# gregspangenberg/shoulder

Hardware: AMD Instinct MI355X
Metric: humerus meshes/s end-to-end (all 4 landmarks) (higher is better)
Workload: dtype f64 geometry + bf16 UNet

## Files before the change

### shoulder_amd/csrc/k_unet16_pp.h

```cpp
#pragma once
#include <type_traits>
#include "k_unet16_base.h"

namespace sh {

#define PP_THREADS 512
#define PP_GTHREADS 256
#define PP_NPIECE 11
#define PP_BUFB (PP_NPIECE * 4096)
#define PP_K1 11
#define PP_G1PRIO 0
#define PP_OFFPRIO 0

template <int N> __device__ inline void pp_wait_vm() {
  if constexpr (N == 0) asm volatile("s_waitcnt vmcnt(0)" ::: "memory");
  else if constexpr (N == 1) asm volatile("s_waitcnt vmcnt(1)" ::: "memory");
  else if constexpr (N == 2) asm volatile("s_waitcnt vmcnt(2)" ::: "memory");
  else if constexpr (N == 3) asm volatile("s_waitcnt vmcnt(3)" ::: "memory");
  else if constexpr (N == 4) asm volatile("s_waitcnt vmcnt(4)" ::: "memory");
  else if constexpr (N == 5) asm volatile("s_waitcnt vmcnt(5)" ::: "memory");
  else if constexpr (N == 6) asm volatile("s_waitcnt vmcnt(6)" ::: "memory");
  else if constexpr (N == 7) asm volatile("s_waitcnt vmcnt(7)" ::: "memory");
  else if constexpr (N == 8) asm volatile("s_waitcnt vmcnt(8)" ::: "memory");
  else if constexpr (N == 9) asm volatile("s_waitcnt vmcnt(9)" ::: "memory");
// ... 634 lines not shown
  const int xh = wv & 1, rg4 = wv >> 1;
  const int ltid = tid & (PP_GTHREADS - 1);
  const int H2 = H >> 1, W2 = W >> 1;
  const int tiles_x = W / 32, tiles_y = H / 8;
  if (tid == 0) { s_q[0] = ud_take_ticket(ticket); s_q[1] = ud_take_ticket(ticket); }

  for (int e = tid; e < 2 * 9 * 32 * 4; e += PP_THREADS) {
    const int row = e >> 2, q = e & 3;
    const int cc = row / 288, rem = row - cc * 288, tap = rem >> 5, j = rem & 31;
    const int ch = 8 * ((j & 15) >> 2) + 4 * (j >> 4) + (j & 3);
    *(u32x4*)(smem + DA_W + e * 16) = *(const u32x4*)(wgt + (size_t)((tap * 2 + cc) * 32 + ch) * 32 + ((q ^ ((row >> 1) & 2)) << 3));
  }
  v8 uw[2][2];
  f32x4 bv[2], ub[2];
#pragma unroll
  for (int kc = 0; kc < 2; ++kc)
#pragma unroll
    for (int n = 0; n < 2; ++n) {
      u32x4 t = *(const u32x4*)(wup + (size_t)((wv * 2 + kc) * 32 + 8 * (li >> 2) + 4 * n + (li & 3)) * 32 + 8 * lk);
      pp_settle(t);
      uw[kc][n] = __builtin_bit_cast(v8, t);
    }
#pragma unroll
  for (int n = 0; n < 2; ++n) {
#pragma unroll
    for (int r = 0; r < 4; ++r) { bv[n][r] = bias[8 * lk + 4 * n + r]; ub[n][r] = upb[8 * lk + 4 * n + r]; }
    pp_settle(bv[n]); pp_settle(ub[n]);
  }
  __syncthreads();
  const int t0 = __builtin_amdgcn_readfirstlane(s_q[0]);
  asm volatile("s_waitcnt vmcnt(0) lgkmcnt(0)" ::: "memory");
  __syncthreads();

  PpCursor cu;
  if (t0 >= ntk) return;
  auto decode = [&](int w) __attribute__((always_inline)) { cu.ty = w % tiles_y; w /= tiles_y; cu.tx = w % tiles_x; cu.img = w / tiles_x; };
  cu.w = tk_tab[t0]; cu.wend = tk_tab[t0 + 1]; cu.qk = 1; cu.live = true;
  decode(cu.w);
  auto advance = [&](const bool fetcher) __attribute__((always_inline)) {
    if (cu.w + 1 < cu.wend) { ++cu.w; if (++cu.ty == tiles_y) { cu.ty = 0; if (++cu.tx == tiles_x) { cu.tx = 0; ++cu.img; } } return; }
    const int nt = __builtin_amdgcn_readfirstlane(s_q[cu.qk]);
    if (nt < ntk) {
      if (fetcher) s_q[cu.qk ^ 1] = ud_take_ticket(ticket);
      cu.qk ^= 1;
      cu.w = tk_tab[nt]; cu.wend = tk_tab[nt + 1];
      decode(cu.w);
    } else cu.live = false;
  };

  const unsigned lds0 = __builtin_amdgcn_readfirstlane((unsigned)(size_t)(ud_lptr)smem);
  const unsigned wv1024 = (unsigned)(wv * 1024);
  int svoff[DA_NSP], lvoff[DA_NLP];
  const int sq8 = ((ltid & 3) ^ (((ltid >> 2) >> 1) & 2)) * 8;
#pragma unroll
  for (int k = 0; k < DA_NSP; ++k) {
    const int r = (ltid >> 2) + 64 * k, py = r / UD_PW, px = r - py * UD_PW;
    svoff[k] = (r < DA_ROWS && px < 34) ? ((py * W + px) * 32 + sq8) * 2 : ((W + 1) * 32 + sq8) * 2;
  }
#pragma unroll
  for (int k = 0; k < DA_NLP; ++k) {
    const int e = ltid + 256 * k, c = e >= 4 * DA_LROWS ? 1 : 0, rem = e - c * 4 * DA_LROWS, lr = rem >> 2;
    const int a = lr / 18, b = lr - a * 18;
    lvoff[k] = (c * (H2 * W2) + a * W2 + b) * 64 + (((rem & 3) ^ ((lr >> 1) & 2)) << 4);
  }
  const bool s5 = (ltid >> 2) + 64 * 5 < DA_ROWS, l3 = ltid + 256 * 3 < 2 * 4 * DA_LROWS;
  auto stage_skip = [&](int bf) __attribute__((always_inline)) {
    const ET* simg = skip + (size_t)cu.img * H * W * 32;
    const unsigned lb = lds0 + (unsigned)(bf * DA_HB) + wv1024;
    if (cu.tx > 0 && cu.tx + 1 < tiles_x && cu.ty > 0 && cu.ty + 1 < tiles_y) {
      const ET* base = simg + ((size_t)(cu.ty * 8 - 1) * W + (cu.tx * 32 - 1)) * 32;
#pragma unroll
      for (int k = 0; k < DA_NSP; ++k)
        if (k < DA_NSP - 1 || s5) ud_dma16_s(lb + k * 4096, (unsigned)svoff[k], base);
    } else {
#pragma unroll
      for (int k = 0; k < DA_NSP; ++k) {
        const int r = (ltid >> 2) + 64 * k, py = r / UD_PW, px = r - py * UD_PW;
        const int gx = cu.tx * 32 + px - 1, gy = cu.ty * 8 + py - 1;
        const bool ok = px < 34 && gx >= 0 && gx < W && gy >= 0 && gy < H;
        const ET* p = ok ? simg + (unsigned)((gy * W + gx) * 32 + sq8) : zero_page;
        if (k < DA_NSP - 1 || s5) ud_dma16(lb + k * 4096, p);
      }
    }
  };
  auto stage_low = [&](int bf) __attribute__((always_inline)) {
    const ET* limg = low + (size_t)cu.img * H2 * W2 * 64;
    const unsigned lb = lds0 + (unsigned)(DA_LOW + bf * DA_LB) + wv1024;
    if (cu.tx > 0 && cu.tx + 1 < tiles_x && cu.ty > 0 && cu.ty + 1 < tiles_y) {
      const ET* base = limg + ((size_t)(cu.ty * 4 - 1) * W2 + (cu.tx * 16 - 1)) * 32;
#pragma unroll
      for (int k = 0; k < DA_NLP; ++k)
        if (k < DA_NLP - 1 || l3) ud_dma16_s(lb + k * 4096, (unsigned)lvoff[k], base);
    } else {
#pragma unroll
      for (int k = 0; k < DA_NLP; ++k) {
        const int e = ltid + 256 * k, c = e >= 4 * DA_LROWS ? 1 : 0, rem = e - c * 4 * DA_LROWS, lr = rem >> 2;
        const int a = lr / 18, b = lr - a * 18;
        const int ly = cu.ty * 4 - 1 + a, lx = cu.tx * 16 - 1 + b;
        const bool ok = ly >= 0 && ly < H2 && lx >= 0 && lx < W2;
        const ET* p = ok ? limg + (size_t)c * H2 * W2 * 32 + (unsigned)((ly * W2 + lx) * 32 + (((rem & 3) ^ ((lr >> 1) & 2)) << 3)) : zero_page;
        if (k < DA_NLP - 1 || l3) ud_dma16(lb + k * 4096, p);
      }
    }
  };
  const int pdy = wv >> 1, pdx = wv & 1;
  int u_low[6], u_out[6];
#pragma unroll
  for (int g = 0; g < 6; ++g) {
    const int t = 16 * g + li;
    const bool valid = t < 85;
    const int a = valid ? t / 17 : 0, bc = valid ? t - a * 17 : 0;
    const int lowrow = (a + (pdy == 0 ? 1 : 0)) * 18 + bc + (pdx == 0 ? 1 : 0);
    const int py = 2 * a + (pdy == 0 ? 1 : 0), px = 2 * bc + (pdx == 0 ? 1 : 0);
    u_low[g] = UB_OFF(lowrow, lk) * 2;
    u_out[g] = valid ? UB_OFF(py * UD_PW + px, lk) * 2 : -1;
  }
  auto upconv = [&](int lb, int ub_, int x0, int y0) __attribute__((always_inline)) {
    const bool interior = x0 > 0 && x0 + 32 < W && y0 > 0 && y0 + 8 < H;
    const unsigned char* lp = smem + DA_LOW + lb * DA_LB;
    unsigned char* op = smem + DA_UP + ub_ * DA_HB;
#pragma unroll
    for (int g0 = 0; g0 < 6; g0 += 3) {
      v8 xf[3][2];
#pragma unroll
      for (int g = 0; g < 3; ++g)
#pragma unroll
        for (int kc = 0; kc < 2; ++kc) xf[g][kc] = *(const v8*)(lp + kc * (DA_LROWS * 64) + u_low[g0 + g]);
      f32x4 ua[3][2];
#pragma unroll
      for (int g = 0; g < 3; ++g)
#pragma unroll
        for (int n = 0; n < 2; ++n) {
          ua[g][n] = ub[n];
#pragma unroll
          for (int kc = 0; kc < 2; ++kc) ua[g][n] = E16<ET>::mfma(uw[kc][n], xf[g][kc], ua[g][n]);
        }
#pragma unroll
      for (int g = 0; g < 3; ++g) {
        u32x4 o;
#pragma unroll
        for (int n = 0; n < 2; ++n) {
          const f32x2 a01 = {ua[g][n][0], ua[g][n][1]}, a23 = {ua[g][n][2], ua[g][n][3]};
          o[2 * n] = __builtin_bit_cast(unsigned, __builtin_convertvector(a01, v2));
          o[2 * n + 1] = __builtin_bit_cast(unsigned, __builtin_convertvector(a23, v2));
        }
        if (!interior) {
          const int t = 16 * (g0 + g) + li, a = t / 17, bc = t - a * 17;
          const int gy = y0 - 1 + 2 * a + (pdy == 0 ? 1 : 0), gx = x0 - 1 + 2 * bc + (pdx == 0 ? 1 : 0);
          if (!(gy >= 0 && gy < H && gx >= 0 && gx < W)) o = u32x4{0u, 0u, 0u, 0u};
        }
        if (u_out[g0 + g] >= 0) *(u32x4*)(op + u_out[g0 + g]) = o;
      }
    }
  };
  int xoff[2][3];
  {
    const int rowbase = rg4 * 4 * UD_PW + xh * 16 + li;
#pragma unroll
    for (int sp = 0; sp < 2; ++sp)
#pragma unroll
      for (int dx = 0; dx < 3; ++dx) xoff[sp][dx] = UB_OFF(rowbase + sp * UD_PW + dx, lk) * 2;
  }
  const int woff = UB_OFF(li, lk) * 2;
  const unsigned so_lane = (unsigned)(((rg4 * 4) * W + xh * 16 + li) * 32 + 8 * lk);

  int ax0 = 0, ay0 = 0, aimg = 0;
  int bx0, by0, bimg; bool blive;
  int cx0, cy0, cimg; bool clive;
  bool alive = false;
  bx0 = cu.tx * 32; by0 = cu.ty * 8; bimg = cu.img; blive = true;
  if (grp == 0) stage_low(0); else stage_skip(0);
  advance(tid == 0);
  asm volatile("s_waitcnt vmcnt(0) lgkmcnt(0)" ::: "memory");
  __builtin_amdgcn_s_barrier();
  asm volatile("" ::: "memory");
  cx0 = cu.tx * 32; cy0 = cu.ty * 8; cimg = cu.img; clive = cu.live;
  if (grp == 0 && cu.live) stage_low(1);
  if (grp == 1) upconv(0, 0, bx0, by0);
  if (cu.live) advance(tid == 0);
  asm volatile("s_waitcnt vmcnt(0) lgkmcnt(0)" ::: "memory");
  __builtin_amdgcn_s_barrier();
  asm volatile("" ::: "memory");

  f32x4 acc[4][2];
#ifdef PP_STAMP
  unsigned long long st_[PP_NSTAMP] = {0, 0, 0, 0, 0, 0, 0, 0};
  PP_T(tl0_);
#endif
  int bf = 0;
  auto phase = [&](const bool on) __attribute__((always_inline)) -> bool {
    if (!blive && !alive) return false;
    PP_T(ta_);
    if (on) {
      if (blive) {
#pragma unroll
        for (int n = 0; n < 2; ++n)
#pragma unroll
          for (int m = 0; m < 4; ++m) acc[m][n] = bv[n];
        if (DA_ONPRIO) __builtin_amdgcn_s_setprio(DA_ONPRIO);
        const unsigned char* sb0 = smem + bf * DA_HB;
        const unsigned char* sb1 = smem + DA_UP + bf * DA_HB;
        const unsigned char* wbp = smem + DA_W + woff;
        v8 xq[2][6], wf[3][2];
        auto tap_of = [](int t) { const int g = t / 3, dy = t % 3; return (g / 3) * 9 + dy * 3 + g % 3; };
#pragma unroll
        for (int s = 0; s < 6; ++s) xq[0][s] = *(const v8*)(sb0 + xoff[s & 1][0] + (s & ~1) * UD_PW * 64);
#pragma unroll
        for (int t = 0; t < 2; ++t)
#pragma unroll
          for (int n = 0; n < 2; ++n) wf[t][n] = *(const v8*)(wbp + (tap_of(t) * 32 + n * 16) * 64);
#pragma unroll
        for (int t = 0; t < 18; ++t) {
          const int g = t / 3, dy = t % 3;
          if (dy == 0 && g + 1 < 6) {
            const unsigned char* sbn = (g + 1) / 3 == 0 ? sb0 : sb1;
#pragma unroll
            for (int s = 0; s < 6; ++s) xq[(g + 1) & 1][s] = *(const v8*)(sbn + xoff[s & 1][(g + 1) % 3] + (s & ~1) * UD_PW * 64);
          }
          if (t + 2 < 18) {
#pragma unroll
            for (int n = 0; n < 2; ++n) wf[(t + 2) % 3][n] = *(const v8*)(wbp + (tap_of(t + 2) * 32 + n * 16) * 64);
          }
          __builtin_amdgcn_sched_barrier(0);
#pragma unroll
          for (int m = 0; m < 4; ++m)
#pragma unroll
            for (int n = 0; n < 2; ++n) acc[m][n] = E16<ET>::mfma(wf[t % 3][n], xq[g & 1][m + dy], acc[m][n]);
          __builtin_amdgcn_sched_barrier(0);
        }
        if (DA_ONPRIO) __builtin_amdgcn_s_setprio(0);
      }
#ifdef PP_STAMP
      asm volatile("" :: "v"(acc[3][1]), "v"(acc[0][0]));
#endif
      PP_T(tb_);
      PP_ADD(0, ta_, tb_);
    } else {
      bool had_stores = false;
      if (clive) {
        const PpCursor keep = cu;
        cu.tx = cx0 >> 5; cu.ty = cy0 >> 3; cu.img = cimg;
        stage_skip(bf ^ 1);
        cu = keep;
      }
      if (cu.live) stage_low(bf);
      PP_T(tb_);
      if (clive) upconv(bf ^ 1, bf ^ 1, cx0, cy0);
      PP_T(tc_);
      PP_ADD(3, ta_, tb_); PP_ADD(1, tb_, tc_);
      if (alive) {
        ET* out = dst + ((size_t)aimg * H * W + (size_t)ay0 * W + ax0) * 32 + so_lane;
        const s16x2 z = {0, 0};
#pragma unroll
        for (int m = 0; m < 4; ++m) {
          u32x4 o;
#pragma unroll
          for (int n = 0; n < 2; ++n) {
            const f32x2 a01 = {acc[m][n][0], acc[m][n][1]}, a23 = {acc[m][n][2], acc[m][n][3]};
            o[2 * n] = __builtin_bit_cast(unsigned, __builtin_elementwise_max(__builtin_bit_cast(s16x2, __builtin_convertvector(a01, v2)), z));
            o[2 * n + 1] = __builtin_bit_cast(unsigned, __builtin_elementwise_max(__builtin_bit_cast(s16x2, __builtin_convertvector(a23, v2)), z));
          }
          ud_store16(out + (size_t)m * W * 32, o);
        }
        had_stores = true;
      }
      if (had_stores) pp_wait_vm<4>(); else pp_wait_vm<0>();
      PP_T(tf_);
      PP_ADD(4, tc_, tf_);
    }
    PP_T(td_);
    ax0 = bx0; ay0 = by0; aimg = bimg; alive = blive;
    bx0 = cx0; by0 = cy0; bimg = cimg; blive = clive;
    cx0 = cu.tx * 32; cy0 = cu.ty * 8; cimg = cu.img; clive = cu.live;
    if (cu.live) advance(on && ltid == 0);
    bf ^= 1;
    asm volatile("s_waitcnt lgkmcnt(0)" ::: "memory");
    __builtin_amdgcn_s_barrier();
    asm volatile("" ::: "memory");
    PP_T(te_);
    PP_ADD(on ? 2 : 5, td_, te_);
#ifdef PP_STAMP
    st_[6] += 1;
#endif
    return true;
  };
  if (PP_G1PRIO && grp == 1) __builtin_amdgcn_s_setprio(PP_G1PRIO);
  if (grp == 0) {
#pragma unroll 1
    for (;;) { if (!phase(true)) break; if (!phase(false)) break; }
  } else {
#pragma unroll 1
    for (;;) { if (!phase(false)) break; if (!phase(true)) break; }
  }
#ifdef PP_STAMP
  {
    PP_T(tl1_);
    st_[7] = tl1_ - tl0_;
    if (lane == 0 && blockIdx.x < 256)
      for (int i = 0; i < PP_NSTAMP; ++i) pp_stamp[(2 * 256 * 8 + blockIdx.x * 8 + wave) * PP_NSTAMP + i] = st_[i];
  }
#endif
}

}
```

### shoulder_amd/csrc/unet.hip

```cpp
#include "sh_ctx.h"

#include "k_unet.h"
#include "k_unet_bf16.h"
#include "k_unet16_ldr.h"
#include "k_unet_x3.h"
#include "k_unet16_up.h"
#include "unet16_pp.h"

using namespace sh;

static int conv_layer(sh_ctx* c, const char* lname, const sh_ctx::ULayer& L, const float* src0, const float* src1, int C0, int C1, float* dst,
                      int H, int W, int nimg, int relu, int fuse = 0, float* pooled = nullptr, const float* head_w = nullptr, const float* head_b = nullptr,
                      float* logits = nullptr, const float* image = nullptr, const float* w0 = nullptr, const float* b0 = nullptr) {
  if (H % UN_TH || W % UN_TW) return fail(c, SH_ERR_ARG, "unet: feature map is not a multiple of 16");
  const float* P = buf<float>(c, "params");
  const float* w = P + L.w_off; const float* b = P + L.b_off;
  const int tiles = (H / UN_TH) * (W / UN_TW);
  if (c->params.unet_dtype == SH_UNET_F32X && C0 % 32 == 0 && C1 % 32 == 0 && L.cout % 32 == 0) {
    const u16* wh = buf<u16>(c, "params_x3h") + L.w_off;
    const u16* wl = buf<u16>(c, "params_x3l") + L.w_off;
    float* np_ = nullptr; const float* nf_ = nullptr;
    if (L.taps == 9 && fuse == (UF_FIRST | UF_POOL) && L.cout == 32 && C0 == 32 && C1 == 0) {
      LAUNCH(c, lname, (k_conv_mfma_x3<9, 2, UF_FIRST | UF_POOL, 0>), dim3(tiles, 1, nimg), dim3(UN_THREADS), src0, src1, C0, C1, wh, wl, b, dst, H, W, L.cout, relu, pooled, nf_, nf_, np_, image, w0, b0);
    }
    else if (L.taps == 9 && fuse == UF_HEAD && L.cout == 32) { LAUNCH(c, lname, (k_conv_mfma_x3<9, 2, UF_HEAD>), dim3(tiles, 1, nimg), dim3(UN_THREADS), src0, src1, C0, C1, wh, wl, b, dst, H, W, L.cout, relu, np_, head_w, head_b, logits, nf_, nf_, nf_); }
    else if (L.taps == 9 && fuse == UF_POOL && L.cout % 64 == 0) { LAUNCH(c, lname, (k_conv_mfma_x3<9, 4, UF_POOL>), dim3(tiles, L.cout / 64, nimg), dim3(UN_THREADS), src0, src1, C0, C1, wh, wl, b, dst, H, W, L.cout, relu, pooled, nf_, nf_, np_, nf_, nf_, nf_); }
    else if (L.taps == 9 && fuse == UF_POOL) { LAUNCH(c, lname, (k_conv_mfma_x3<9, 2, UF_POOL, 0>), dim3(tiles, L.cout / 32, nimg), dim3(UN_THREADS), src0, src1, C0, C1, wh, wl, b, dst, H, W, L.cout, relu, pooled, nf_, nf_, np_, nf_, nf_, nf_); }
    else if (fuse != 0) return fail(c, SH_ERR_ARG, "unet: unsupported fusion");
    else if (L.taps == 9 && L.cout % 64 == 0) { LAUNCH(c, lname, (k_conv_mfma_x3<9, 4>), dim3(tiles, L.cout / 64, nimg), dim3(UN_THREADS), src0, src1, C0, C1, wh, wl, b, dst, H, W, L.cout, relu, np_, nf_, nf_, np_, nf_, nf_, nf_); }
    else if (L.taps == 9) { LAUNCH(c, lname, (k_conv_mfma_x3<9, 2, 0, 0>), dim3(tiles, L.cout / 32, nimg), dim3(UN_THREADS), src0, src1, C0, C1, wh, wl, b, dst, H, W, L.cout, relu, np_, nf_, nf_, np_, nf_, nf_, nf_); }
    else if (C1 == 0 && W % 32 == 0 && H % 16 == 0 && (C0 == 64 || C0 == 128 || C0 == 256 || C0 == 512)) {
      if (C0 == 64) { LAUNCH(c, lname, (k_upconv_x3r<2, 4>), dim3((W / 32) * (H / 16), nimg), dim3(UXR_THREADS), src0, wh, wl, b, dst, H, W, L.cout); }
      else if (C0 == 128) { LAUNCH(c, lname, (k_upconv_x3r<4, 4>), dim3((W / 32) * (H / 16), nimg), dim3(UXR_THREADS), src0, wh, wl, b, dst, H, W, L.cout); }
      else if (C0 == 256) { LAUNCH(c, lname, (k_upconv_x3r<8, 2>), dim3((W / 32) * (H / 8), nimg), dim3(UXR_THREADS), src0, wh, wl, b, dst, H, W, L.cout); }
      else { LAUNCH(c, lname, (k_upconv_x3r<16, 1>), dim3((W / 32) * (H / 4), nimg), dim3(UXR_THREADS), src0, wh, wl, b, dst, H, W, L.cout); }
    }
    else if (L.cout % 64 == 0) { LAUNCH(c, lname, (k_conv_mfma_x3<1, 4>), dim3(tiles, L.cout / 64, nimg * 4), dim3(UN_THREADS), src0, src1, C0, C1, wh, wl, b, dst, H, W, L.cout, 0, np_, nf_, nf_, np_, nf_, nf_, nf_); }
    else { LAUNCH(c, lname, (k_conv_mfma_x3<1, 2>), dim3(tiles, L.cout / 32, nimg * 4), dim3(UN_THREADS), src0, src1, C0, C1, wh, wl, b, dst, H, W, L.cout, 0, np_, nf_, nf_, np_, nf_, nf_, nf_); }
    return SH_OK;
  }
  if (L.taps == 9) {
    if (L.cout % 64 == 0) {
      LAUNCH(c, lname, (k_conv_mfma_f32<9, 4>), dim3(tiles, L.cout / 64, nimg), dim3(UN_THREADS), src0, src1, C0, C1, w, b, dst, H, W, L.cout, relu);
    } else {
      LAUNCH(c, lname, (k_conv_mfma_f32<9, 2>), dim3(tiles, L.cout / 32, nimg), dim3(UN_THREADS), src0, src1, C0, C1, w, b, dst, H, W, L.cout, relu);
    }
  } else {
    if (L.cout % 64 == 0) {
      LAUNCH(c, lname, (k_conv_mfma_f32<1, 4>), dim3(tiles, L.cout / 64, nimg * 4), dim3(UN_THREADS), src0, src1, C0, C1, w, b, dst, H, W, L.cout, 0);
    } else {
      LAUNCH(c, lname, (k_conv_mfma_f32<1, 2>), dim3(tiles, L.cout / 32, nimg * 4), dim3(UN_THREADS), src0, src1, C0, C1, w, b, dst, H, W, L.cout, 0);
    }
  }
  return SH_OK;
}

static std::mutex g_turn_mu;
static hipEvent_t g_turn_last[64] = {};
static sh_ctx* g_turn_owner[64] = {};

namespace sh {

int unet_turn_enter(sh_ctx* c) {
  if (!c->unet_turn || c->device < 0 || c->device >= 64) return SH_OK;
  std::lock_guard<std::mutex> lk(g_turn_mu);
  if (g_turn_last[c->device] && g_turn_owner[c->device] != c) HIPCHK(c, hipStreamWaitEvent(c->stream, g_turn_last[c->device], 0));
  return SH_OK;
}

int unet_turn_leave(sh_ctx* c) {
  if (!c->unet_turn || c->device < 0 || c->device >= 64) return SH_OK;
  std::lock_guard<std::mutex> lk(g_turn_mu);
  if (!c->unet_done_ev) HIPCHK(c, hipEventCreateWithFlags(&c->unet_done_ev, hipEventDisableTiming));
  HIPCHK(c, hipEventRecord(c->unet_done_ev, c->stream));
  g_turn_last[c->device] = c->unet_done_ev;
  g_turn_owner[c->device] = c;
  return SH_OK;
}

void unet_turn_forget(sh_ctx* c) {
  std::lock_guard<std::mutex> lk(g_turn_mu);
  if (c->device >= 0 && c->device < 64 && g_turn_owner[c->device] == c) { g_turn_last[c->device] = nullptr; g_turn_owner[c->device] = nullptr; }
}

}

static int unet_forward(sh_ctx* c, const float* image, float* logits, int nimg, int H, int W) {
  const int D = c->unet_depth, base = c->unet_base;
  if ((H >> D) % 16 || (W >> D) % 16) return fail(c, SH_ERR_ARG, "unet: input size must be a multiple of 16 << depth");
  int rc;
  const size_t full = (size_t)nimg * H * W * base * 4;
  if ((rc = ensure(c, "unet.a", full, 4)) != SH_OK) return rc;
  if ((rc = ensure(c, "unet.b", full, 4)) != SH_OK) return rc;
  std::vector<float*> skip(D);
  for (int i = 0; i < D; ++i) {
    std::string nm = "unet.skip" + std::to_string(i);
    if ((rc = ensure(c, nm.c_str(), full >> i, 4)) != SH_OK) return rc;
    skip[i] = buf<float>(c, nm.c_str());
  }
  float* A = buf<float>(c, "unet.a");
  float* Bq = buf<float>(c, "unet.b");
  const float* P = buf<float>(c, "params");
  if (c->params.unet_dtype == SH_UNET_F32X) {
    if ((rc = ensure(c, "params_x3h", c->unet_floats * 2, 2)) != SH_OK) return rc;
    if ((rc = ensure(c, "params_x3l", c->unet_floats * 2, 2)) != SH_OK) return rc;
    if (!c->packed_x3) {
      std::vector<PackEntry> tab;
      long long total = 0;
      for (auto& kv : c->ulayers) {
        const sh_ctx::ULayer& l = kv.second;
        if (l.cin < 32 || l.cout < 32) continue;
        tab.push_back(PackEntry{total, (long long)l.w_off, l.taps, l.cin, l.cout, 0});
        total += (long long)l.taps * l.cin * l.cout;
        if (c->h_unet.size() >= l.w_off + (size_t)l.taps * l.cin * l.cout) {
          const float* wl = c->h_unet.data() + l.w_off;
          for (size_t i = 0, n = (size_t)l.taps * l.cin * l.cout; i < n; ++i)
            if (!(fabsf(wl[i]) < 65504.0f / X3_WSCALE)) {
              char m[200];
              snprintf(m, sizeof m, "SH_UNET_F32X: layer %s has a weight of magnitude %g; the split-f16 operands hold |w| < %g (use SH_UNET_F32 for this network)",
                       kv.first.c_str(), (double)fabsf(wl[i]), (double)(65504.0f / X3_WSCALE));
              return fail(c, SH_ERR_ARG, m);
            }
        }
      }
      if ((rc = ensure(c, "unet16.packtab", tab.size() * sizeof(PackEntry), 8)) != SH_OK) return rc;
      HIPCHK(c, hipMemcpyAsync(c->bufs["unet16.packtab"].p, tab.data(), tab.size() * sizeof(PackEntry), hipMemcpyHostToDevice, c->stream));
      HIPCHK(c, hipStreamSynchronize(c->stream));
      c->packtab_ready = true;
      LAUNCH(c, "k_pack_w_x3", k_pack_w_x3, dim3(2048), dim3(256), P, buf<u16>(c, "params_x3h"), buf<u16>(c, "params_x3l"), (const PackEntry*)c->bufs["unet16.packtab"].p, (int)tab.size(), total);
      c->packed_x3 = true;
    }
  }
  auto L = [&](const std::string& n) -> const sh_ctx::ULayer& { return c->ulayers[n]; };
  int h = H, w = W;
  const bool x3 = c->params.unet_dtype == SH_UNET_F32X && base % 32 == 0;
  const bool x3_first = x3 && base == 32;
  if (!x3_first) {
    const sh_ctx::ULayer& l = L("enc0a");
    size_t npx = (size_t)nimg * h * w;
    LAUNCH(c, "unet.enc0a", k_conv_first, dim3((unsigned)std::min<size_t>((npx + 255) / 256, 8192)), dim3(256), image, P + l.w_off, P + l.b_off, A, h, w, l.cout, nimg);
  }
  if (x3_first) {
    const sh_ctx::ULayer& l = L("enc0a");
    if ((rc = conv_layer(c, "unet.enc0b", L("enc0b"), A, nullptr, base, 0, skip[0], h, w, nimg, 1, UF_FIRST | UF_POOL, Bq, nullptr, nullptr, nullptr, image, P + l.w_off, P + l.b_off)) != SH_OK) return rc;
  } else if ((rc = conv_layer(c, "unet.enc0b", L("enc0b"), A, nullptr, base, 0, skip[0], h, w, nimg, 1, x3 ? UF_POOL : 0, Bq)) != SH_OK) return rc;
  if (x3) std::swap(A, Bq);
  int ch = base;
  for (int i = 1; i <= D; ++i) {
    if (!x3) {
      size_t e = (size_t)nimg * (h / 2) * (w / 2) * (ch / 4);
      LAUNCH(c, "unet.pool", k_maxpool2, dim3((unsigned)std::min<size_t>((e + 255) / 256, 8192)), dim3(256), skip[i - 1], A, h, w, ch, nimg);
    }
    h /= 2; w /= 2;
    std::string na = i < D ? "enc" + std::to_string(i) + "a" : "bota", nb = i < D ? "enc" + std::to_string(i) + "b" : "botb";
    if ((rc = conv_layer(c, ("unet." + na).c_str(), L(na), A, nullptr, ch, 0, Bq, h, w, nimg, 1)) != SH_OK) return rc;
    ch *= 2;
    float* dst = i < D ? skip[i] : A;
    if ((rc = conv_layer(c, ("unet." + nb).c_str(), L(nb), Bq, nullptr, ch, 0, dst, h, w, nimg, 1, (x3 && i < D) ? UF_POOL : 0, A)) != SH_OK) return rc;
  }
  float* x = A; float* y = Bq;
  for (int i = D - 1; i >= 0; --i) {
    std::string nu = "up" + std::to_string(i), na = "dec" + std::to_string(i) + "a", nb = "dec" + std::to_string(i) + "b";
    if ((rc = conv_layer(c, ("unet." + nu).c_str(), L(nu), x, nullptr, ch, 0, y, h, w, nimg, 0)) != SH_OK) return rc;
    h *= 2; w *= 2; ch /= 2;
    if ((rc = conv_layer(c, ("unet." + na).c_str(), L(na), skip[i], y, ch, ch, x, h, w, nimg, 1)) != SH_OK) return rc;
    if ((rc = conv_layer(c, ("unet." + nb).c_str(), L(nb), x, nullptr, ch, 0, y, h, w, nimg, 1)) != SH_OK) return rc;
    std::swap(x, y);
  }
  {
    const sh_ctx::ULayer& l = L("head");
    size_t npx = (size_t)nimg * H * W;
    if (l.cin <= 32) { LAUNCH(c, "unet.head", k_head<32>, dim3((unsigned)std::min<size_t>((npx + 255) / 256, 16384)), dim3(256), x, P + l.w_off, P + l.b_off, logits, l.cin, npx); }
    else { LAUNCH(c, "unet.head", k_head<64>, dim3((unsigned)std::min<size_t>((npx + 255) / 256, 8192)), dim3(256), x, P + l.w_off, P + l.b_off, logits, l.cin, npx); }
  }
  return SH_OK;
}

#define SH_UNET_TICKETS 64
#define SH_UNET_TKTAB (1 << 18)
static int persistent_grid(sh_ctx* c) {
  constexpr int cu_reserve = 32;
  if (c->num_cus <= 0) { int v = 0; if (hipDeviceGetAttribute(&v, hipDeviceAttributeMultiprocessorCount, c->device) != hipSuccess) v = 0; c->num_cus = v > 0 ? v : 256; }
  return c->unet_turn ? std::max(8, c->num_cus - cu_reserve) : c->num_cus;
}

static int unet_tickets(sh_ctx* c, int total, int nwg, int ngrp, unsigned** tk, const int** tk_tab, int* ntk) {
  const auto key = std::make_tuple(total, nwg, ngrp);
  auto it = c->tk_tabs.find(key);
  if (it == c->tk_tabs.end()) {
    std::vector<int> tab;
    int pos = 0;
    while (pos < total) {
      int sz = std::max(1, (int)std::ceil((total - pos) / (3.0 * (double)nwg)));
      if (sz >= ngrp) sz = sz / ngrp * ngrp;
      tab.push_back(pos);
      pos += std::min(sz, total - pos);
    }
    tab.push_back(total);
    if ((int)tab.size() > SH_UNET_TKTAB) return fail(c, SH_ERR_CAPACITY, "unet: ticket table larger than its buffer");
    if (c->tk_tab_used + (int)tab.size() > SH_UNET_TKTAB) {
      HIPCHK(c, hipStreamSynchronize(c->stream));
      c->tk_tabs.clear();
      c->tk_tab_used = 0;
    }
    HIPCHK(c, hipMemcpyAsync(buf<int>(c, "unet16.tk_tab") + c->tk_tab_used, tab.data(), tab.size() * 4, hipMemcpyHostToDevice, c->stream));
    HIPCHK(c, hipStreamSynchronize(c->stream));
    it = c->tk_tabs.emplace(key, std::make_pair(c->tk_tab_used, (int)tab.size() - 1)).first;
    c->tk_tab_used += (int)tab.size();
  }
  if (c->ticket_next >= SH_UNET_TICKETS) return fail(c, SH_ERR_CAPACITY, "unet: out of work counters");
  *tk = buf<unsigned>(c, "unet16.tickets") + c->ticket_next++;
  *tk_tab = buf<int>(c, "unet16.tk_tab") + it->second.first;
  *ntk = it->second.second;
  return SH_OK;
}

template <int EK>
static int conv_layer16(sh_ctx* c, const char* lname, const sh_ctx::ULayer& L, const u16* src0, const u16* src1, int C0, int C1,
                           u16* dst, int H, int W, int nimg, int relu, int fuse = 0, ConvFuse fz = ConvFuse{}) {
  if (H % UN_TH || W % UN_TW) return fail(c, SH_ERR_ARG, "unet: feature map is not a multiple of 16");
  const u16* w = buf<u16>(c, "params_bf16") + L.w_off;
  const float* b = buf<float>(c, "params") + L.b_off;
  const int tiles = (H / UN_TH) * (W / UN_TW);
  const dim3 blk(UN_THREADS);
  const bool ldr = !c->unet_reference && L.taps == 9 && L.cout % 64 == 0 && L.cout <= 512 && W % 32 == 0 && H % 16 == 0 && C0 % 32 == 0 && C1 % 32 == 0 &&
                   (fuse == 0 || (fuse == UF_POOL && relu));
  if (ldr) {
    int rc0;
    if ((rc0 = ensure(c, "unet16.zero", 256, 2)) != SH_OK) return rc0;
    if (!c->zero_page_ready) { HIPCHK(c, hipMemsetAsync(buf<char>(c, "unet16.zero"), 0, 256, c->stream)); c->zero_page_ready = true; }
    const int total = nimg * (W / 32) * (H / 16) * (L.cout / 64);
    const dim3 g((unsigned)std::min(total, persistent_grid(c)));
    unsigned* tk = nullptr; const int* tk_tab = nullptr; int ntk = 0;
    if ((rc0 = unet_tickets(c, total, (int)g.x, L.cout / 64, &tk, &tk_tab, &ntk)) != SH_OK) return rc0;
    const u16* zp = (const u16*)c->bufs["unet16.zero"].p;
    u16* pl = fuse == UF_POOL ? (u16*)fz.pooled : (u16*)nullptr;
    const bool wres = L.cout == 64 && ((C0 + C1) / 32) * 64 <= 128;
    if (fuse == UF_POOL && wres) { LAUNCH(c, lname, (k_conv3_ldr16<EK, UF_POOL, 1>), g, dim3(UD_THREADS), src0, src1, C0, C1, w, b, dst, H, W, L.cout, relu, nimg, zp, pl, tk, tk_tab, ntk); }
    else if (fuse == UF_POOL) { LAUNCH(c, lname, (k_conv3_ldr16<EK, UF_POOL, 0>), g, dim3(UD_THREADS), src0, src1, C0, C1, w, b, dst, H, W, L.cout, relu, nimg, zp, pl, tk, tk_tab, ntk); }
    else if (wres) { LAUNCH(c, lname, (k_conv3_ldr16<EK, 0, 1>), g, dim3(UD_THREADS), src0, src1, C0, C1, w, b, dst, H, W, L.cout, relu, nimg, zp, pl, tk, tk_tab, ntk); }
    else { LAUNCH(c, lname, (k_conv3_ldr16<EK, 0, 0>), g, dim3(UD_THREADS), src0, src1, C0, C1, w, b, dst, H, W, L.cout, relu, nimg, zp, pl, tk, tk_tab, ntk); }
  } else if (L.taps == 9 && L.cout % 64 == 0) {
    const dim3 g(tiles, L.cout / 64, nimg);
    if (fuse == 0) { LAUNCH(c, lname, (k_conv_mfma16<EK, 9, 4, 0>), g, blk, src0, src1, C0, C1, w, b, dst, H, W, L.cout, relu, fz); }
    else if (fuse == UF_POOL) { LAUNCH(c, lname, (k_conv_mfma16<EK, 9, 4, UF_POOL>), g, blk, src0, src1, C0, C1, w, b, dst, H, W, L.cout, relu, fz); }
    else return fail(c, SH_ERR_ARG, "unet: unsupported fusion");
  } else if (L.taps == 9) {
    const dim3 g(tiles, L.cout / 32, nimg);
    if (fuse == 0) { LAUNCH(c, lname, (k_conv_mfma16<EK, 9, 2, 0>), g, blk, src0, src1, C0, C1, w, b, dst, H, W, L.cout, relu, fz); }
    else return fail(c, SH_ERR_ARG, "unet: unsupported fusion");
  } else if (!c->unet_reference && L.cout % 32 == 0 && C1 == 0 && C0 % 32 == 0) {
    const bool upg = W % 32 == 0 && H % 16 == 0 && (C0 == 128 || C0 == 256 || C0 == 512) && L.cout <= 512;
    if (upg) {
      const int mt = C0 == 128 ? 4 : 2, nitems = (W / 32) * (H / (4 * mt)) * nimg;
      const int grid = C0 == 512 ? nitems : std::min(nitems, persistent_grid(c));
      unsigned* tk = nullptr; const int* tk_tab = nullptr; int ntk = 0;
      if (C0 != 512) { const int trc = unet_tickets(c, nitems, grid, 1, &tk, &tk_tab, &ntk); if (trc != SH_OK) return trc; }
      if (C0 == 128) { LAUNCH(c, lname, (k_upconv16g<EK, 4, 4, 4, true>), dim3((unsigned)grid), dim3(UPR_THREADS), src0, w, b, dst, H, W, L.cout, nimg, tk, tk_tab, ntk); }
      else if (C0 == 256) { LAUNCH(c, lname, (k_upconv16g<EK, 8, 2, 4, true>), dim3((unsigned)grid), dim3(UPR_THREADS), src0, w, b, dst, H, W, L.cout, nimg, tk, tk_tab, ntk); }
      else { LAUNCH(c, lname, (k_upconv16g<EK, 16, 2, 2, false>), dim3((unsigned)grid), dim3(UPR_THREADS), src0, w, b, dst, H, W, L.cout, nimg, tk, tk_tab, ntk); }
    }
    else { LAUNCH(c, lname, (k_upconv16<EK>), dim3(tiles, L.cout / 32, nimg * 2), dim3(UPC_THREADS), src0, C0, w, b, dst, H, W, L.cout); }
  } else if (L.cout % 64 == 0) {
    LAUNCH(c, lname, (k_conv_mfma16<EK, 1, 4, 0>), dim3(tiles, L.cout / 64, nimg * 4), blk, src0, src1, C0, C1, w, b, dst, H, W, L.cout, 0, fz);
  } else {
    LAUNCH(c, lname, (k_conv_mfma16<EK, 1, 2, 0>), dim3(tiles, L.cout / 32, nimg * 4), blk, src0, src1, C0, C1, w, b, dst, H, W, L.cout, 0, fz);
  }
  return SH_OK;
}

namespace sh {
bool unet16_level0_fused(const sh_ctx* c, int H, int W) {
  return !c->unet_reference && c->unet_base == 32 && c->unet_depth >= 1 && W % 32 == 0 && H % 16 == 0 && (H >> c->unet_depth) % 16 == 0 && (W >> c->unet_depth) % 16 == 0;
}
}

template <int EK>
static int unet_forward16(sh_ctx* c, const float* image, float* logits, int nimg, int H, int W) {
  const int D = c->unet_depth, base = c->unet_base;
  if ((H >> D) % 16 || (W >> D) % 16) return fail(c, SH_ERR_ARG, "unet: input size must be a multiple of 16 << depth");
  int rc;
  if ((rc = ensure(c, "params_bf16", c->unet_floats * 2, 2)) != SH_OK) return rc;
  const float* P = buf<float>(c, "params");
  u16* PW = buf<u16>(c, "params_bf16");
  if (c->packed_kind != EK) {
    std::vector<PackEntry> tab;
    long long total = 0;
    for (auto& kv : c->ulayers) {
      const sh_ctx::ULayer& l = kv.second;
      if (l.cin < 32 || l.cout < 32) continue;
      tab.push_back(PackEntry{total, (long long)l.w_off, l.taps, l.cin, l.cout, 0});
      total += (long long)l.taps * l.cin * l.cout;
    }
    if ((rc = ensure(c, "unet16.packtab", tab.size() * sizeof(PackEntry), 8)) != SH_OK) return rc;
    if (!c->packtab_ready) {
      HIPCHK(c, hipMemcpyAsync(c->bufs["unet16.packtab"].p, tab.data(), tab.size() * sizeof(PackEntry), hipMemcpyHostToDevice, c->stream));
      HIPCHK(c, hipStreamSynchronize(c->stream));
      c->packtab_ready = true;
    }
    LAUNCH(c, "k_pack_w_bf16", k_pack_w16_all<EK>, dim3(2048), dim3(256), P, PW, (const PackEntry*)c->bufs["unet16.packtab"].p, (int)tab.size(), total);
    c->packed_kind = EK;
  }
  if ((rc = ensure(c, "unet16.tickets", SH_UNET_TICKETS * 4, 4)) != SH_OK) return rc;
  if ((rc = ensure(c, "unet16.tk_tab", SH_UNET_TKTAB * 4, 4)) != SH_OK) return rc;
  FILL(c, {buf<unsigned>(c, "unet16.tickets"), (size_t)SH_UNET_TICKETS * 4, 0});
  c->ticket_next = 0;
  const bool fused = unet16_level0_fused(c, H, W);
  const size_t full = (size_t)nimg * H * W * base * 2;
  if ((rc = ensure(c, "unet16.a", full, 2)) != SH_OK) return rc;
  if ((rc = ensure(c, "unet16.b", full, 2)) != SH_OK) return rc;
  std::vector<u16*> skip(D);
  for (int i = 0; i < D; ++i) {
    std::string nm = "unet16.skip" + std::to_string(i);
    if ((rc = ensure(c, nm.c_str(), full >> i, 2)) != SH_OK) return rc;
    skip[i] = buf<u16>(c, nm.c_str());
  }
  u16* A = buf<u16>(c, "unet16.a");
  u16* Bq = buf<u16>(c, "unet16.b");
  auto L = [&](const std::string& n) -> const sh_ctx::ULayer& { return c->ulayers[n]; };
  if ((rc = ensure(c, "unet16.zero", 256, 2)) != SH_OK) return rc;
  if (!c->zero_page_ready) { HIPCHK(c, hipMemsetAsync(buf<char>(c, "unet16.zero"), 0, 256, c->stream)); c->zero_page_ready = true; }
  const u16* zp = (const u16*)c->bufs["unet16.zero"].p;
  int h = H, w = W;
  if (fused) {
    const sh_ctx::ULayer& la = L("enc0a");
    const sh_ctx::ULayer& lb = L("enc0b");
    const int total = nimg * (w / 32) * (h / 16);
    const unsigned grid = (unsigned)std::min(total, persistent_grid(c));
    unsigned* tk = nullptr; const int* tk_tab = nullptr; int ntk = 0;
    if ((rc = unet_tickets(c, total, (int)grid, 1, &tk, &tk_tab, &ntk)) != SH_OK) return rc;
    LAUNCH_FN(c, "unet.enc0b", launch_enc0_pp(EK, grid, c->stream, image, P + la.w_off, P + la.b_off, PW + lb.w_off, P + lb.b_off, skip[0], A, h, w, nimg,
                                              c->unet_raw, c->unet_mm, tk, tk_tab, ntk));
  } else {
    const sh_ctx::ULayer& l = L("enc0a");
    size_t npx = (size_t)nimg * h * w;
    LAUNCH(c, "unet.enc0a", k_conv_first16<EK>, dim3((unsigned)std::min<size_t>((npx + 255) / 256, 8192)), dim3(256), image, P + l.w_off, P + l.b_off, A, h, w, l.cout, nimg);
    if ((rc = conv_layer16<EK>(c, "unet.enc0b", L("enc0b"), A, nullptr, base, 0, skip[0], h, w, nimg, 1)) != SH_OK) return rc;
  }
  int ch = base;
  for (int i = 1; i <= D; ++i) {
    if (!fused) {
      size_t e = (size_t)nimg * (h / 2) * (w / 2) * (ch / 8);
      LAUNCH(c, "unet.pool", k_maxpool2_16<EK>, dim3((unsigned)std::min<size_t>((e + 255) / 256, 8192)), dim3(256), skip[i - 1], A, h, w, ch, nimg);
    }
    h /= 2; w /= 2;
    std::string na = i < D ? "enc" + std::to_string(i) + "a" : "bota", nb = i < D ? "enc" + std::to_string(i) + "b" : "botb";
    if ((rc = conv_layer16<EK>(c, ("unet." + na).c_str(), L(na), A, nullptr, ch, 0, Bq, h, w, nimg, 1)) != SH_OK) return rc;
    ch *= 2;
    u16* dst = i < D ? skip[i] : A;
    ConvFuse fz{};
    fz.pooled = A;
    if ((rc = conv_layer16<EK>(c, ("unet." + nb).c_str(), L(nb), Bq, nullptr, ch, 0, dst, h, w, nimg, 1, (fused && i < D) ? UF_POOL : 0, fz)) != SH_OK) return rc;
  }
  u16* x = A; u16* y = Bq;
  for (int i = D - 1; i >= 0; --i) {
    std::string nu = "up" + std::to_string(i), na = "dec" + std::to_string(i) + "a", nb = "dec" + std::to_string(i) + "b";
    if (fused && i == 0) {
      h *= 2; w *= 2; ch /= 2;
      const sh_ctx::ULayer& lu = L(nu);
      const sh_ctx::ULayer& la = L(na);
      const sh_ctx::ULayer& lb = L(nb);
      const sh_ctx::ULayer& lh = L("head");
      {
        const int total = nimg * (w / 32) * (h / 8);
        const unsigned grid = (unsigned)std::min(total, persistent_grid(c));
        unsigned* tk = nullptr; const int* tk_tab = nullptr; int ntk = 0;
        if ((rc = unet_tickets(c, total, (int)grid, 1, &tk, &tk_tab, &ntk)) != SH_OK) return rc;
        LAUNCH_FN(c, "unet.dec0a", launch_dec0a_up_pp(EK, grid, c->stream, skip[0], x, PW + la.w_off, P + la.b_off, PW + lu.w_off, P + lu.b_off, y, h, w, nimg,
                                                      zp, tk, tk_tab, ntk));
      }
      {
        const int total = nimg * (w / 32) * (h / 16);
        const unsigned grid = (unsigned)std::min(total, persistent_grid(c));
        unsigned* tk = nullptr; const int* tk_tab = nullptr; int ntk = 0;
        if ((rc = unet_tickets(c, total, (int)grid, 1, &tk, &tk_tab, &ntk)) != SH_OK) return rc;
        LAUNCH_FN(c, "unet.dec0b", launch_dec0b_head_pp(EK, grid, c->stream, y, PW + lb.w_off, P + lb.b_off, P + lh.w_off, P + lh.b_off, logits, h, w, nimg,
                                                        zp, tk, tk_tab, ntk));
      }
      return SH_OK;
    }
    if ((rc = conv_layer16<EK>(c, ("unet." + nu).c_str(), L(nu), x, nullptr, ch, 0, y, h, w, nimg, 0)) != SH_OK) return rc;
    h *= 2; w *= 2; ch /= 2;
    if ((rc = conv_layer16<EK>(c, ("unet." + na).c_str(), L(na), skip[i], y, ch, ch, x, h, w, nimg, 1)) != SH_OK) return rc;
    if ((rc = conv_layer16<EK>(c, ("unet." + nb).c_str(), L(nb), x, nullptr, ch, 0, y, h, w, nimg, 1)) != SH_OK) return rc;
    std::swap(x, y);
  }
  {
    const sh_ctx::ULayer& l = L("head");
    size_t npx = (size_t)nimg * H * W;
    LAUNCH(c, "unet.head", k_head16<EK>, dim3((unsigned)std::min<size_t>((npx + 255) / 256, 8192)), dim3(256), x, P + l.w_off, P + l.b_off, logits, l.cin, npx, (size_t)H * W);
  }
  return SH_OK;
}

namespace sh {
int unet_dispatch(sh_ctx* c, const float* image, float* logits, int nimg, int H, int W) {
  switch (c->params.unet_dtype) {
    case SH_UNET_BF16: return unet_forward16<0>(c, image, logits, nimg, H, W);
    case SH_UNET_F16: return unet_forward16<1>(c, image, logits, nimg, H, W);
    default: return unet_forward(c, image, logits, nimg, H, W);
  }
}
}

extern "C" {

int sh_unet_infer(sh_ctx* c, const float* images, int n, int H, int W, float* logits) {
  if (!c || !images || !logits || n <= 0 || H <= 0 || W <= 0) return fail(c, SH_ERR_ARG, "sh_unet_infer: bad argument");
  if (c->ulayers.empty()) return fail(c, SH_ERR_STATE, "sh_unet_infer: no UNet weights loaded");
  HIPCHK(c, hipSetDevice(c->device));
  const size_t bytes = (size_t)n * H * W * 4;
  int rc;
  if ((rc = ensure(c, "infer.image", bytes, 4)) != SH_OK) return rc;
  if ((rc = ensure(c, "infer.logits", bytes, 4)) != SH_OK) return rc;
  WindowScope whole(c, 0, c->Bwin);
  HIPCHK(c, hipMemcpyAsync(buf<float>(c, "infer.image"), images, bytes, hipMemcpyHostToDevice, c->stream));
  rc = unet_dispatch(c, buf<float>(c, "infer.image"), buf<float>(c, "infer.logits"), n, H, W);
  if (rc != SH_OK) { (void)hipStreamSynchronize(c->stream); return rc; }
  HIPCHK(c, hipMemcpyAsync(logits, buf<float>(c, "infer.logits"), bytes, hipMemcpyDeviceToHost, c->stream));
  HIPCHK(c, hipStreamSynchronize(c->stream));
  return SH_OK;
}

}
```

### shoulder_amd/csrc/unet16_pp.h

```cpp
#pragma once
#include <hip/hip_runtime.h>

namespace sh {

void launch_dec0b_head_pp(int ek, unsigned grid, hipStream_t st, const unsigned short* src, const unsigned short* wgt, const float* bias,
                          const float* head_w, const float* head_b, float* logits, int H, int W, int nimg, const unsigned short* zero_page,
                          unsigned* ticket, const int* tk_tab, int ntk);

void launch_enc0_pp(int ek, unsigned grid, hipStream_t st, const float* image, const float* w0, const float* b0, const unsigned short* wgt,
                    const float* bias, unsigned short* skip, unsigned short* pooled, int H, int W, int nimg, const double* raw,
                    const unsigned long long* mm, unsigned* ticket, const int* tk_tab, int ntk);

void launch_dec0a_up_pp(int ek, unsigned grid, hipStream_t st, const unsigned short* skip, const unsigned short* low, const unsigned short* wgt,
                        const float* bias, const unsigned short* wup, const float* upb, unsigned short* dst, int H, int W, int nimg,
                        const unsigned short* zero_page, unsigned* ticket, const int* tk_tab, int ntk);

}
```

### shoulder_amd/csrc/unet16_pp.hip

```cpp
#include "k_unet16_pp.h"
#include "unet16_pp.h"

namespace sh {

void launch_dec0b_head_pp(int ek, unsigned grid, hipStream_t st, const unsigned short* src, const unsigned short* wgt, const float* bias,
                          const float* head_w, const float* head_b, float* logits, int H, int W, int nimg, const unsigned short* zero_page,
                          unsigned* ticket, const int* tk_tab, int ntk) {
  if (ek == 0) hipLaunchKernelGGL((k_dec0b_head_pp<0>), dim3(grid), dim3(PP_THREADS), 0, st, src, wgt, bias, head_w, head_b, logits, H, W, nimg, zero_page, ticket, tk_tab, ntk);
  else hipLaunchKernelGGL((k_dec0b_head_pp<1>), dim3(grid), dim3(PP_THREADS), 0, st, src, wgt, bias, head_w, head_b, logits, H, W, nimg, zero_page, ticket, tk_tab, ntk);
}

void launch_enc0_pp(int ek, unsigned grid, hipStream_t st, const float* image, const float* w0, const float* b0, const unsigned short* wgt,
                    const float* bias, unsigned short* skip, unsigned short* pooled, int H, int W, int nimg, const double* raw,
                    const unsigned long long* mm, unsigned* ticket, const int* tk_tab, int ntk) {
#define E0_GO(EK, RAW) hipLaunchKernelGGL((k_enc0_pp<EK, RAW>), dim3(grid), dim3(PP_THREADS), 0, st, image, w0, b0, wgt, bias, skip, pooled, H, W, nimg, raw, mm, ticket, tk_tab, ntk)
  if (ek == 0) { if (raw) E0_GO(0, true); else E0_GO(0, false); }
  else { if (raw) E0_GO(1, true); else E0_GO(1, false); }
#undef E0_GO
}

}

namespace sh {
void launch_dec0a_up_pp(int ek, unsigned grid, hipStream_t st, const unsigned short* skip, const unsigned short* low, const unsigned short* wgt,
                        const float* bias, const unsigned short* wup, const float* upb, unsigned short* dst, int H, int W, int nimg,
                        const unsigned short* zero_page, unsigned* ticket, const int* tk_tab, int ntk) {
  if (ek == 0) hipLaunchKernelGGL((k_dec0a_up_pp<0>), dim3(grid), dim3(PP_THREADS), 0, st, skip, low, wgt, bias, wup, upb, dst, H, W, nimg, zero_page, ticket, tk_tab, ntk);
  else hipLaunchKernelGGL((k_dec0a_up_pp<1>), dim3(grid), dim3(PP_THREADS), 0, st, skip, low, wgt, bias, wup, upb, dst, H, W, nimg, zero_page, ticket, tk_tab, ntk);
}
}

#ifdef PP_STAMP
extern "C" int sh_lab_pp_stamps(unsigned long long* out) {
  return (int)hipMemcpyFromSymbol(out, HIP_SYMBOL(sh::pp_stamp), sizeof(unsigned long long) * 3 * 256 * 8 * PP_NSTAMP);
}
#endif
```

Before: 9157.

## Add ping-pong persistent conv kernel for 64-channel level-1 UNet convs

Result: no change. 9138 (-0.2%).

```diff
diff --git a/shoulder_amd/csrc/k_unet16_pp.h b/shoulder_amd/csrc/k_unet16_pp.h
--- a/shoulder_amd/csrc/k_unet16_pp.h
+++ b/shoulder_amd/csrc/k_unet16_pp.h
@@ -960,4 +960,222 @@
 #endif
 }
 
+
+#define L1_HB (UD_INROWS * 64)
+#define L1_WOFF (2 * L1_HB)
+#define L1_WCH (9 * 64 * 64)
+#define L1_BIAS (L1_WOFF + 2 * L1_WCH)
+#define L1_SMEM (L1_BIAS + 256)
+#ifndef L1_OFFPRIO
+#define L1_OFFPRIO 0
+#endif
+#define L1_NPIECE 11
+
+template <int N> __device__ inline void l1_wait_vm() { asm volatile("s_waitcnt vmcnt(%0)" :: "n"(N) : "memory"); }
+
+template <int EK, bool POOL>
+__global__ void __launch_bounds__(PP_THREADS)
+k_conv3_l1pp(const u16* __restrict__ src_ , int Cin , const u16* __restrict__ wgt_ ,
+             const float* __restrict__ bias, u16* __restrict__ dst_ , u16* __restrict__ pooled_ ,
+             int H, int W, int nimg, const u16* __restrict__ zero_page_, unsigned* __restrict__ ticket, const int* __restrict__ tk_tab, int ntk) {
+  using ET = typename EKT<EK>::type;
+  using v8 = typename E16<ET>::v8;
+  using v2 = typename E16<ET>::v2;
+  typedef float f32x2 __attribute__((ext_vector_type(2)));
+  const ET* src = (const ET*)src_;
+  const ET* wgt = (const ET*)wgt_;
+  ET* dst = (ET*)dst_;
+  ET* pooled = (ET*)pooled_;
+  const ET* zero_page = (const ET*)zero_page_;
+  constexpr int NST = POOL ? 24 : 16;
+  __shared__ __attribute__((aligned(1024))) unsigned char smem[L1_SMEM];
+  __shared__ int s_q[2];
+  const int tid = threadIdx.x, lane = tid & 63, wave = tid >> 6;
+  const int li = lane & 15, lk = lane >> 4;
+  const int grp = __builtin_amdgcn_readfirstlane(wave >> 2), wv = __builtin_amdgcn_readfirstlane(wave & 3);
+  const int xh = wv & 1, rg8 = wv >> 1;
+  const int ltid = tid & (PP_GTHREADS - 1);
+  const int nchunk = Cin >> 5;
+  const int tiles_x = W / 32, tiles_y = H / 16;
+  if (tid == 0) { s_q[0] = ud_take_ticket(ticket); s_q[1] = ud_take_ticket(ticket); }
+
+  float* s_bias = (float*)(smem + L1_BIAS);
+  if (tid < 64) s_bias[tid] = bias[tid];
+  for (int e = tid; e < nchunk * 9 * 64 * 4; e += PP_THREADS) {
+    const int row = e >> 2, q = e & 3;
+    const int cc = row / (9 * 64), rem = row - cc * 9 * 64, tap = rem >> 6, j = rem & 63;
+    const int ch = 16 * ((j & 15) >> 2) + 4 * (j >> 4) + (j & 3);
+    *(u32x4*)(smem + L1_WOFF + e * 16) = *(const u32x4*)(wgt + (size_t)((tap * nchunk + cc) * 64 + ch) * 32 + ((q ^ ((row >> 1) & 2)) << 3));
+  }
+  asm volatile("s_waitcnt vmcnt(0) lgkmcnt(0)" ::: "memory");
+  __syncthreads();
+  int qk = 1;
+  int w, w_end;
+  {
+    const int t0 = __builtin_amdgcn_readfirstlane(s_q[0]);
+    if (t0 >= ntk) return;
+    w = tk_tab[t0]; w_end = tk_tab[t0 + 1];
+  }
+  int i_tx, i_ty, i_img;
+  auto decode = [&](int v) { i_tx = v % tiles_x; v /= tiles_x; i_ty = v % tiles_y; i_img = v / tiles_y; };
+  decode(w);
+  w = __builtin_amdgcn_readfirstlane(w); w_end = __builtin_amdgcn_readfirstlane(w_end);
+  i_tx = __builtin_amdgcn_readfirstlane(i_tx); i_ty = __builtin_amdgcn_readfirstlane(i_ty); i_img = __builtin_amdgcn_readfirstlane(i_img);
+  auto walk = [&](int cc, int& n_cc, bool& has_next, bool& more, const bool fetcher) __attribute__((always_inline)) {
+    n_cc = cc + 1;
+    has_next = true;
+    if (n_cc < nchunk) {
+    } else if (w + 1 < w_end) {
+      ++w;
+      if (++i_tx == tiles_x) { i_tx = 0; if (++i_ty == tiles_y) { i_ty = 0; ++i_img; } }
+      n_cc = 0;
+    } else {
+      const int nt = __builtin_amdgcn_readfirstlane(s_q[qk]);
+      if (nt < ntk) {
+        if (fetcher) s_q[qk ^ 1] = ud_take_ticket(ticket);
+        qk ^= 1;
+        w = tk_tab[nt]; w_end = tk_tab[nt + 1];
+        decode(w);
+        n_cc = 0;
+      } else { has_next = false; more = false; }
+    }
+    i_tx = __builtin_amdgcn_readfirstlane(i_tx); i_ty = __builtin_amdgcn_readfirstlane(i_ty); i_img = __builtin_amdgcn_readfirstlane(i_img);
+    w = __builtin_amdgcn_readfirstlane(w); w_end = __builtin_amdgcn_readfirstlane(w_end);
+    n_cc = __builtin_amdgcn_readfirstlane(n_cc);
+  };
+
+  const unsigned lds0 = __builtin_amdgcn_readfirstlane((unsigned)(size_t)(ud_lptr)smem);
+  const int r0 = ltid >> 2;
+  const int q8 = ((ltid & 3) ^ ((r0 >> 1) & 2)) * 8;
+  const bool tail = r0 < 8;
+  auto stage = [&](int cc, int buf) __attribute__((always_inline)) {
+    const ET* simg = src + ((size_t)i_img * nchunk + cc) * H * W * 32;
+    const unsigned lbase = lds0 + (unsigned)(buf * L1_HB) + (unsigned)(wv * 1024);
+    int r0v = r0;
+#pragma unroll
+    for (int k = 0; k < L1_NPIECE; ++k) {
+      asm volatile("" : "+v"(r0v));
+      const int r = r0v + 64 * k, hpy = r / UD_PW, hpx = r - hpy * UD_PW;
+      const int gx = i_tx * 32 + hpx - 1, gy = i_ty * 16 + hpy - 1;
+      const bool in = hpx < 34 && gx >= 0 && gx < W && gy >= 0 && gy < H;
+      const ET* p = in ? simg + (unsigned)((gy * W + gx) * 32 + q8) : zero_page;
+      if (k < L1_NPIECE - 1) ud_dma16(lbase + k * 4096, p);
+      else if (tail) ud_dma16(lbase + k * 4096, p);
+    }
+  };
+
+  int xoff[2][3];
+  {
+    const int rowbase = rg8 * 8 * UD_PW + xh * 16 + li;
+#pragma unroll
+    for (int sp = 0; sp < 2; ++sp)
+#pragma unroll
+      for (int dx = 0; dx < 3; ++dx) xoff[sp][dx] = UB_OFF(rowbase + sp * UD_PW + dx, lk) * 2;
+  }
+  const int woff = UB_OFF(li, lk) * 2;
+  auto multiply = [&](f32x4 (&acc)[8][4], int cc, int buf) __attribute__((always_inline)) {
+    const unsigned char* sb = smem + buf * L1_HB;
+    const unsigned char* wbp = smem + L1_WOFF + cc * L1_WCH + woff;
+#pragma unroll
+    for (int dx = 0; dx < 3; ++dx) {
+      v8 xq[10];
+#pragma unroll
+      for (int s = 0; s < 10; ++s) xq[s] = *(const v8*)(sb + xoff[s & 1][dx] + (s & ~1) * UD_PW * 64);
+#pragma unroll
+      for (int dy = 0; dy < 3; ++dy) {
+        const int tap = dy * 3 + dx;
+        v8 wf[4];
+#pragma unroll
+        for (int n = 0; n < 4; ++n) wf[n] = *(const v8*)(wbp + (tap * 64 + n * 16) * 64);
+#pragma unroll
+        for (int m = 0; m < 8; ++m)
+#pragma unroll
+          for (int n = 0; n < 4; ++n) acc[m][n] = E16<ET>::mfma(wf[n], xq[m + dy], acc[m][n]);
+      }
+    }
+  };
+  auto epilogue = [&](const f32x4 (&acc)[8][4], int c_x0, int c_y0, int c_img) __attribute__((always_inline)) {
+    const unsigned HW = (unsigned)(H * W);
+    ET* ob = dst + (size_t)c_img * 64 * HW;
+    const unsigned lo = (((unsigned)(lk >> 1) * HW + (unsigned)((c_y0 + rg8 * 8) * W + c_x0 + xh * 16 + li)) << 5) + 16u * (lk & 1);
+    ET* pb = pooled;
+    unsigned plo = 0;
+    if (POOL) {
+      pb = pooled + (size_t)c_img * 64 * (HW >> 2);
+      plo = (((unsigned)(lk >> 1) * (HW >> 2) + (unsigned)(((c_y0 + rg8 * 8) >> 1) * (W >> 1) + ((c_x0 + xh * 16 + li) >> 1))) << 5) + 16u * (lk & 1);
+    }
+#pragma unroll
+    for (int mp = 0; mp < 4; ++mp)
+#pragma unroll
+      for (int h = 0; h < 2; ++h) {
+        unsigned lo_ = lo, plo_ = plo;
+        asm volatile("" : "+v"(lo_), "+v"(plo_));
+        u32x4 ua, ub;
+#pragma unroll
+        for (int i = 0; i < 4; ++i) {
+          const f32x4& ra = acc[2 * mp][2 * h + (i >> 1)];
+          const f32x4& rb = acc[2 * mp + 1][2 * h + (i >> 1)];
+          const f32x2 pa = {ra[2 * (i & 1)], ra[2 * (i & 1) + 1]}, pb2 = {rb[2 * (i & 1)], rb[2 * (i & 1) + 1]};
+          ua[i] = pp_pkmax(__builtin_bit_cast(unsigned, __builtin_convertvector(pa, v2)), 0u);
+          ub[i] = pp_pkmax(__builtin_bit_cast(unsigned, __builtin_convertvector(pb2, v2)), 0u);
+        }
+        ud_store16(ob + (lo_ + (unsigned)((2 * mp) * W * 32 + 8 * h)), ua);
+        ud_store16(ob + (lo_ + (unsigned)((2 * mp + 1) * W * 32 + 8 * h)), ub);
+        if (POOL) {
+          u32x4 pv;
+#pragma unroll
+          for (int i = 0; i < 4; ++i) pv[i] = pp_pkmax_lane1(pp_pkmax(ua[i], ub[i]));
+          if (!(li & 1)) ud_store16(pb + (plo_ + (unsigned)(mp * (W >> 1) * 32 + 8 * h)), pv);
+        }
+      }
+  };
+
+  if (grp == 1) stage(0, 0);
+  f32x4 acc[8][4];
+  int e_x0 = 0, e_y0 = 0, e_img = 0;
+  bool pending = false;
+  bool stored = false;
+  bool more = true;
+  int buf = 0;
+  auto item = [&](const bool on) __attribute__((always_inline)) -> bool {
+    if (on) {
+      e_x0 = i_tx * 32; e_y0 = i_ty * 16; e_img = i_img;
+#pragma unroll
+      for (int n = 0; n < 4; ++n) {
+        const f32x4 bv = *(const f32x4*)(s_bias + 16 * lk + 4 * n);
+#pragma unroll
+        for (int m = 0; m < 8; ++m) acc[m][n] = bv;
+      }
+    }
+#pragma unroll 1
+    for (int cc = 0; cc < nchunk; ++cc) {
+      if (stored) l1_wait_vm<NST>(); else l1_wait_vm<0>();
+      stored = false;
+      asm volatile("s_waitcnt lgkmcnt(0)" ::: "memory");
+      __builtin_amdgcn_s_barrier();
+      asm volatile("" ::: "memory");
+      int n_cc; bool has_next;
+      walk(cc, n_cc, has_next, more, on && ltid == 0);
+      if (on) multiply(acc, cc, buf);
+      else {
+        if (L1_OFFPRIO) __builtin_amdgcn_s_setprio(L1_OFFPRIO);
+        if (has_next) stage(n_cc, buf ^ 1);
+        if (cc == 0 && pending) { epilogue(acc, e_x0, e_y0, e_img); pending = false; stored = true; }
+        if (L1_OFFPRIO) __builtin_amdgcn_s_setprio(0);
+      }
+      buf ^= 1;
+    }
+    if (on) pending = true;
+    return more;
+  };
+  if (grp == 0) {
+#pragma unroll 1
+    for (;;) { if (!item(true)) break; if (!item(false)) break; }
+  } else {
+#pragma unroll 1
+    for (;;) { if (!item(false)) break; if (!item(true)) break; }
+  }
+  if (pending) epilogue(acc, e_x0, e_y0, e_img);
 }
+
+}
diff --git a/shoulder_amd/csrc/unet.hip b/shoulder_amd/csrc/unet.hip
--- a/shoulder_amd/csrc/unet.hip
+++ b/shoulder_amd/csrc/unet.hip
@@ -235,10 +235,9 @@
     if ((rc0 = unet_tickets(c, total, (int)g.x, L.cout / 64, &tk, &tk_tab, &ntk)) != SH_OK) return rc0;
     const u16* zp = (const u16*)c->bufs["unet16.zero"].p;
     u16* pl = fuse == UF_POOL ? (u16*)fz.pooled : (u16*)nullptr;
-    const bool wres = L.cout == 64 && ((C0 + C1) / 32) * 64 <= 128;
-    if (fuse == UF_POOL && wres) { LAUNCH(c, lname, (k_conv3_ldr16<EK, UF_POOL, 1>), g, dim3(UD_THREADS), src0, src1, C0, C1, w, b, dst, H, W, L.cout, relu, nimg, zp, pl, tk, tk_tab, ntk); }
+    const bool l1pp = L.cout == 64 && C1 == 0 && (C0 == 32 || C0 == 64) && relu;
+    if (l1pp) { LAUNCH_FN(c, lname, launch_conv3_l1pp(EK, fuse == UF_POOL, g.x, c->stream, src0, C0, w, b, dst, pl, H, W, nimg, zp, tk, tk_tab, ntk)); }
     else if (fuse == UF_POOL) { LAUNCH(c, lname, (k_conv3_ldr16<EK, UF_POOL, 0>), g, dim3(UD_THREADS), src0, src1, C0, C1, w, b, dst, H, W, L.cout, relu, nimg, zp, pl, tk, tk_tab, ntk); }
-    else if (wres) { LAUNCH(c, lname, (k_conv3_ldr16<EK, 0, 1>), g, dim3(UD_THREADS), src0, src1, C0, C1, w, b, dst, H, W, L.cout, relu, nimg, zp, pl, tk, tk_tab, ntk); }
     else { LAUNCH(c, lname, (k_conv3_ldr16<EK, 0, 0>), g, dim3(UD_THREADS), src0, src1, C0, C1, w, b, dst, H, W, L.cout, relu, nimg, zp, pl, tk, tk_tab, ntk); }
   } else if (L.taps == 9 && L.cout % 64 == 0) {
     const dim3 g(tiles, L.cout / 64, nimg);
diff --git a/shoulder_amd/csrc/unet16_pp.h b/shoulder_amd/csrc/unet16_pp.h
--- a/shoulder_amd/csrc/unet16_pp.h
+++ b/shoulder_amd/csrc/unet16_pp.h
@@ -15,4 +15,8 @@
                         const float* bias, const unsigned short* wup, const float* upb, unsigned short* dst, int H, int W, int nimg,
                         const unsigned short* zero_page, unsigned* ticket, const int* tk_tab, int ntk);
 
+void launch_conv3_l1pp(int ek, bool pool, unsigned grid, hipStream_t st, const unsigned short* src, int Cin, const unsigned short* wgt, const float* bias,
+                       unsigned short* dst, unsigned short* pooled, int H, int W, int nimg, const unsigned short* zero_page,
+                       unsigned* ticket, const int* tk_tab, int ntk);
+
 }
diff --git a/shoulder_amd/csrc/unet16_pp.hip b/shoulder_amd/csrc/unet16_pp.hip
--- a/shoulder_amd/csrc/unet16_pp.hip
+++ b/shoulder_amd/csrc/unet16_pp.hip
@@ -30,6 +30,17 @@
 }
 }
 
+namespace sh {
+void launch_conv3_l1pp(int ek, bool pool, unsigned grid, hipStream_t st, const unsigned short* src, int Cin, const unsigned short* wgt, const float* bias,
+                       unsigned short* dst, unsigned short* pooled, int H, int W, int nimg, const unsigned short* zero_page,
+                       unsigned* ticket, const int* tk_tab, int ntk) {
+#define L1_GO(EK, POOL) hipLaunchKernelGGL((k_conv3_l1pp<EK, POOL>), dim3(grid), dim3(PP_THREADS), 0, st, src, Cin, wgt, bias, dst, pooled, H, W, nimg, zero_page, ticket, tk_tab, ntk)
+  if (ek == 0) { if (pool) L1_GO(0, true); else L1_GO(0, false); }
+  else { if (pool) L1_GO(1, true); else L1_GO(1, false); }
+#undef L1_GO
+}
+}
+
 #ifdef PP_STAMP
 extern "C" int sh_lab_pp_stamps(unsigned long long* out) {
   return (int)hipMemcpyFromSymbol(out, HIP_SYMBOL(sh::pp_stamp), sizeof(unsigned long long) * 3 * 256 * 8 * PP_NSTAMP);
```
